# pdishuck/GAVISUNK

Measured on NVIDIA B200. Metric: ont_read_gbp_per_s_sunk_matched_validated, higher is better.
Workload: dtype u64

## Files before the change

gavisunk_b200/csrc/probe.cu:

```cuda
#include "table.cuh"
#include <stdlib.h>
#include <vector>

#ifndef PW_WARPS
#define PW_WARPS 8
#endif
#ifndef PW_BLOCKS
#define PW_BLOCKS 4
#endif
#define PW_TILE 512
static_assert(PW_TILE == GVS_TILE_BASES, "ctx.cu sizes the copy segments in probe tiles");
#define PW_RING 64
#define PW_MAXB 32

#define FLAG_KEYERROR 1u
#define FLAG_OVERFLOW 2u

__device__ __forceinline__ u32 p_codes4(u32 x) {
  u32 f = ((x >> 1) ^ (x >> 2)) & 0x03030303u;
  u32 l = x | 0x20202020u;
  u32 letter = __vcmpeq4(l, 0x63636363u) | __vcmpeq4(l, 0x67676767u) | __vcmpeq4(l, 0x74747474u) |
               __vcmpeq4(l, 0x75757575u);
  u32 low = __vcmpeq4(x & 0xFCFCFCFCu, 0u);
  return (f & letter) | (x & low & 0x03030303u);
}
__device__ __forceinline__ u32 p_codes4_fast(u32 x, u32& bad) {
  u32 f = ((x >> 1) ^ (x >> 2)) & 0x03030303u;
  u32 t = f | (f >> 4);
  u32 sel = __byte_perm(t, 0u, 0x4420);
  u32 letters = __byte_perm(0x54474341u, 0u, sel);
  bad |= letters ^ (x & 0xDFDFDFDFu);
  return f;
}
__device__ __forceinline__ u32 p_be8_top(u32 c) { return c * 0x40100401u; }
__device__ __forceinline__ u32 p_gather_top(u32 px, u32 py, u32 pz, u32 pw) {
  u32 t1 = __byte_perm(py, px, 0x0073);
  u32 t2 = __byte_perm(pw, pz, 0x0073);
  return __byte_perm(t2, t1, 0x5410);
}
__device__ __forceinline__ u32 p_pack16_be(uint4 v) {
  return p_gather_top(p_be8_top(p_codes4(v.x)), p_be8_top(p_codes4(v.y)), p_be8_top(p_codes4(v.z)), p_be8_top(p_codes4(v.w)));
}
__device__ __forceinline__ u32 p_pack16_be_fast(uint4 v, u32& bad) {
  return p_gather_top(p_be8_top(p_codes4_fast(v.x, bad)), p_be8_top(p_codes4_fast(v.y, bad)),
                      p_be8_top(p_codes4_fast(v.z, bad)), p_be8_top(p_codes4_fast(v.w, bad)));
}
__device__ __forceinline__ u32 p_rc16(u32 w) {
  u32 x = __brev(~w);
  return ((x >> 1) & 0x55555555u) | ((x & 0x55555555u) << 1);
}
template <int LEN>
__device__ __forceinline__ u64 p_extract(u32 a, u32 b, u32 c, int off) {
  int s = 2 * off;
  u32 hi = __funnelshift_l(b, a, s);
  u32 lo = __funnelshift_l(c, b, s);
  u64 v = ((u64)hi << 32) | lo;
  return v >> (64 - 2 * LEN);
}

struct __align__(16) WarpSmem {
  u32 fw[PW_RING];
  u32 rc[PW_RING];
  uint4 raw[32];
  u64 bar;
  u32 bound[20];
  u32 shrt[20];
  u32 bpos[PW_MAXB];
  u32 bidx[PW_MAXB];
  u32 cand[PW_TILE / 32];
  u16 inv[32];
  u32 q_row[PW_TILE];
  u16 q_p[PW_TILE];
  u32 s_blk[32][3];
  u16 s_p[32];
};

template <int K>
__device__ __forceinline__ u64 p_fwd_at(const WarpSmem& sm, u32 rb, u32 p) {
  u32 wi = rb + (p >> 4);
  return p_extract<K>(sm.fw[wi & 63], sm.fw[(wi + 1) & 63], sm.fw[(wi + 2) & 63], p & 15);
}
template <int K>
__device__ __forceinline__ u64 p_rc_at(const WarpSmem& sm, u32 rb, u32 p) {
  u32 e = p + K, c = (e + 15) >> 4;
  u32 wi = rb + c - 1;
  return p_extract<K>(sm.rc[wi & 63], sm.rc[(wi - 1) & 63], sm.rc[(wi - 2) & 63], 16 * c - e);
}
template <int K>
__device__ __forceinline__ u64 p_canon_at(const WarpSmem& sm, u32 rb, u32 p, bool force_last_a) {
  u64 f = p_fwd_at<K>(sm, rb, p), r = p_rc_at<K>(sm, rb, p);
  if (force_last_a) {
    f &= ~3ull;
    r |= 3ull << (2 * (K - 1));
  }
  return f < r ? f : r;
}

struct Probe2Params {
  const u8* __restrict__ seq;
  u64 total;
  const u64* __restrict__ read_off;
  u64 n_reads;
  u64 tile_begin, tile_stop;
  u64 span_base;
  u32 span_tiles, n_spans;
  u32* span_ctr;
  u32 blk_stream;
  const u32* __restrict__ filt;
  u32 filt_mask;
  const u32* __restrict__ filt1;
  u32 filt1_words;
  TabView tab;
  u32* hit_read;
  u32* hit_w;
  u32* hit_row;
  u32* hit_gidx;
  u8* hit_nf;
  u64 hit_cap;
  u32* flags;
  u32* warp_cnt;
  u64 cap_w;
};

__device__ __forceinline__ u64 p_policy_stream() {
  u64 p;
  asm volatile("createpolicy.fractional.L2::evict_first.b64 %0, 1.0;" : "=l"(p));
  return p;
}
__device__ __forceinline__ u64 p_policy_keep() {
  u64 p;
  asm volatile("createpolicy.fractional.L2::evict_last.b64 %0, 1.0;" : "=l"(p));
  return p;
}
__device__ __forceinline__ uint4 p_ldg_v4(const uint4* ptr, u64 pol) {
  uint4 v;
  asm volatile("ld.global.nc.L2::cache_hint.L2::64B.v4.u32 {%0,%1,%2,%3}, [%4], %5;"
               : "=r"(v.x), "=r"(v.y), "=r"(v.z), "=r"(v.w)
               : "l"(ptr), "l"(pol));
  return v;
}
__device__ __forceinline__ u32 p_ldg_u32(const u32* ptr, u64 pol) {
  u32 v;
  asm volatile("ld.global.nc.L2::cache_hint.L2::64B.u32 %0, [%1], %2;" : "=r"(v) : "l"(ptr), "l"(pol));
  return v;
}

__device__ __forceinline__ u32 p_smem_addr(const void* p) { return (u32)__cvta_generic_to_shared(p); }
__device__ __forceinline__ void p_bar_init(u64* bar) {
  asm volatile("mbarrier.init.shared::cta.b64 [%0], 1;\n" ::"r"(p_smem_addr(bar)) : "memory");
  asm volatile("fence.mbarrier_init.release.cluster;\n" ::: "memory");
}
__device__ __forceinline__ void p_bar_wait(u64* bar, u32 phase) {
  asm volatile(
      "{\n"
      ".reg .pred p;\n"
      "PW_WAIT:\n"
      "mbarrier.try_wait.parity.shared::cta.b64 p, [%0], %1;\n"
      "@p bra PW_DONE;\n"
      "bra PW_WAIT;\n"
      "PW_DONE:\n"
      "}\n" ::"r"(p_smem_addr(bar)),
      "r"(phase)
      : "memory");
}
template <bool PACKED>
__device__ __forceinline__ u32 p_tile_bytes(u64 tile, u64 total) {
  const u64 unit = PACKED ? PW_TILE / 4 : PW_TILE;
  const u64 have = PACKED ? 4 * ((total + 15) >> 4) : total;
  const u64 b0 = tile * unit;
  if (b0 >= have) return 0;
  const u64 r = have - b0;
  return r >= unit ? (u32)unit : (u32)((r + 15) & ~15ull);
}
template <bool PACKED, bool FULL = false>
__device__ __forceinline__ void p_stage_issue(WarpSmem& sm, const u8* __restrict__ seq, u64 tile, u64 total, int lane, u64 pol) {
  const u32 bytes = FULL ? (PACKED ? PW_TILE / 4 : PW_TILE) : p_tile_bytes<PACKED>(tile, total);
  if (lane == 0 && bytes) {
    const u32 bar = p_smem_addr(&sm.bar), dst = p_smem_addr(&sm.raw[0]);
    const u8* src = seq + tile * (PACKED ? PW_TILE / 4 : PW_TILE);
    asm volatile("fence.proxy.async.shared::cta;\n" ::: "memory");
    asm volatile("mbarrier.arrive.expect_tx.shared::cta.b64 _, [%0], %1;\n" ::"r"(bar), "r"(bytes) : "memory");
    asm volatile("cp.async.bulk.shared::cluster.global.mbarrier::complete_tx::bytes.L2::cache_hint [%0], [%1], %2, [%3], %4;\n" ::"r"(dst),
                 "l"(src), "r"(bytes), "r"(bar), "l"(pol)
                 : "memory");
  }
}
template <bool PACKED, bool FULL = false>
__device__ __forceinline__ void p_stage_finish(WarpSmem& sm, u32 rb, u64 tile, u64 total, int lane, u32& phase) {
  if (FULL) {
    p_bar_wait(&sm.bar, phase);
    phase ^= 1u;
    u32 w;
    if (PACKED) {
      w = ((const u32*)sm.raw)[lane];
    } else {
      const uint4 v = sm.raw[lane];
      u32 bad = 0;
      w = p_pack16_be_fast(v, bad);
      if (__any_sync(0xFFFFFFFFu, bad != 0)) w = p_pack16_be(v);
    }
    sm.fw[(rb + lane) & 63] = w;
    sm.rc[(rb + lane) & 63] = p_rc16(w);
    return;
  }
  const u32 bytes = p_tile_bytes<PACKED>(tile, total);
  if (bytes) {
    p_bar_wait(&sm.bar, phase);
    phase ^= 1u;
  }
  u32 w = 0;
  if (PACKED) {
    if (4u * lane < bytes) w = ((const u32*)sm.raw)[lane];
  } else {
    uint4 v = make_uint4(0u, 0u, 0u, 0u);
    const u64 g = tile * PW_TILE + 16ull * lane;
    const bool tail = g + 16 > total;
    if (16u * lane < bytes) {
      v = sm.raw[lane];
      if (tail) {
        const u32 nv = g < total ? (u32)(total - g) : 0u;
        u32 x[4] = {v.x, v.y, v.z, v.w};
#pragma unroll
        for (int i = 0; i < 4; i++) {
          const u32 left = nv > 4u * i ? nv - 4u * i : 0u;
          x[i] &= left >= 4u ? 0xFFFFFFFFu : ((1u << (8 * left)) - 1u);
        }
        v = make_uint4(x[0], x[1], x[2], x[3]);
      }
    }
    u32 bad = 0;
    w = p_pack16_be_fast(v, bad);
    if (__any_sync(0xFFFFFFFFu, (bad != 0) | tail)) w = p_pack16_be(v);
  }
  sm.fw[(rb + lane) & 63] = w;
  sm.rc[(rb + lane) & 63] = p_rc16(w);
}

template <int K, bool PACKED, bool SMALL>
__global__ void __launch_bounds__(PW_WARPS * 32, PW_BLOCKS) k_probe2(const Probe2Params P) {
  __shared__ WarpSmem sm_all[PW_WARPS];
  const int lane = threadIdx.x & 31;
  WarpSmem& sm = sm_all[threadIdx.x >> 5];
  constexpr int CMAX = (K + 15 + 15) / 16;
  constexpr u32 ALL = 0xFFFFFFFFu;
  constexpr int J = GVS_FJ(K);
  constexpr int L = K - J + 1;
  constexpr int NG = 16 / J;
  const u64 pol_keep = p_policy_keep();
  const u64 pol_stream = p_policy_stream();
  const u64 pol_blk = P.blk_stream ? pol_stream : pol_keep;
  if (lane == 0) p_bar_init(&sm.bar);
  __syncwarp();
  u32 phase = 0;

  for (;;) {
    u32 span = 0;
    if (lane == 0) span = atomicAdd(P.span_ctr, 1u);
    span = __shfl_sync(ALL, span, 0);
    if (span >= P.n_spans) break;
    const u64 tile0 = P.tile_begin + (u64)span * P.span_tiles;
    u64 tile_end = tile0 + P.span_tiles;
    if (tile_end > P.tile_stop) tile_end = P.tile_stop;
    const u64 region = P.span_base + span;

    u64 cur;
    {
      u64 ts0 = tile0 * PW_TILE;
      u64 lo = 1, hi = P.n_reads;
      while (lo < hi) {
        u64 mid = (lo + hi) >> 1;
        if (__ldg(P.read_off + mid) > ts0) hi = mid; else lo = mid + 1;
      }
      cur = lo;
    }
    u64 next_off = __ldg(P.read_off + cur);
    u64 prev_off = __ldg(P.read_off + cur - 1);

    __syncwarp();
    p_stage_issue<PACKED>(sm, P.seq, tile0, P.total, lane, pol_stream);
    p_stage_finish<PACKED>(sm, 0, tile0, P.total, lane, phase);
    __syncwarp();
    p_stage_issue<PACKED>(sm, P.seq, tile0 + 1, P.total, lane, pol_stream);
    p_stage_finish<PACKED>(sm, 32, tile0 + 1, P.total, lane, phase);
    __syncwarp();

    const bool span_full = (tile_end + 2) * PW_TILE <= P.total;
    u32 wcount = 0;
    for (u64 tile = tile0; tile < tile_end; tile++) {
      const u64 ts = tile * PW_TILE;
      const u32 rb = (u32)((tile - tile0) & 1) * 32;
      if (span_full) p_stage_issue<PACKED, true>(sm, P.seq, tile + 2, P.total, lane, pol_stream);
      else p_stage_issue<PACKED>(sm, P.seq, tile + 2, P.total, lane, pol_stream);

      const u64 limit = ts + PW_TILE + (K > 1 ? K - 1 : 1);
      const u64 cur0 = cur;
      u32 nb = 0;
      const bool has_bound = next_off < limit;
      const bool start_short = K >= 2 && prev_off == ts && next_off - prev_off == (u64)(K - 1);
      if (has_bound) {
        if (lane < 20) { sm.bound[lane] = 0; sm.shrt[lane] = 0; }
        __syncwarp();
        u64 j = cur + lane;
        for (;;) {
          u64 o = (j <= P.n_reads) ? __ldg(P.read_off + j) : ~0ull;
          bool inr = o < limit;
          bool intile = inr && (o - ts) < PW_TILE;
          u32 bal_tile = __ballot_sync(ALL, intile);
          if (inr) {
            u32 rel = (u32)(o - ts);
            atomicOr(&sm.bound[rel >> 5], 1u << (rel & 31));
            if (intile) {
              u32 slot = nb + __popc(bal_tile & ((1u << lane) - 1));
              if (slot < PW_MAXB) { sm.bpos[slot] = rel; sm.bidx[slot] = (u32)j; }
              if (K >= 2 && j < P.n_reads && __ldg(P.read_off + j + 1) - o == (u64)(K - 1))
                atomicOr(&sm.shrt[rel >> 5], 1u << (rel & 31));
            }
          }
          nb += __popc(bal_tile);
          u32 bal_adv = __ballot_sync(ALL, o <= ts + PW_TILE);
          cur += __popc(bal_adv);
          u32 bal_in = __ballot_sync(ALL, inr);
          if (bal_in != ALL) break;
          j += 32;
        }
        next_off = (cur <= P.n_reads) ? __ldg(P.read_off + cur) : ~0ull;
        prev_off = __ldg(P.read_off + cur - 1);
        __syncwarp();
      }

      u32 cm = 0;
      u32 S16 = 0;
      u32 pass = 0;
      u32 hbv[NG];
      {
        const u32 wb = rb + lane;
        const u32 f0 = sm.fw[wb & 63], f1 = sm.fw[(wb + 1) & 63], f2 = sm.fw[(wb + 2) & 63];
        const u32 r0 = sm.rc[(wb + CMAX - 1) & 63], r1 = sm.rc[(wb + CMAX - 2) & 63], r2 = sm.rc[(wb + CMAX - 3) & 63],
                  r3 = sm.rc[(wb + CMAX - 4) & 63];
        u32 inval = 0;
        if (has_bound) {
          int idx = lane >> 1, sh = (lane & 1) * 16;
          u64 B = ((u64)sm.bound[idx] | ((u64)sm.bound[idx + 1] << 32)) >> sh;
          if (sh) B |= (u64)sm.bound[idx + 2] << 48;
          u64 x = 0;
          if (K >= 2) {
            x = B >> 1;
            int c = 1;
#pragma unroll
            for (int it = 0; it < 6; it++) {
              if (c < K - 1) {
                int step = (K - 1 - c) < c ? (K - 1 - c) : c;
                x |= x >> step;
                c += step;
              }
            }
          }
          inval = (u32)x & 0xFFFFu;
          S16 = (sm.shrt[idx] >> sh) & 0xFFFFu;
        }
        if (start_short && lane == 0) S16 |= 1u;
        {
          u64 p0 = ts + 16ull * lane;
          if (p0 + 16 > P.total) {
            u32 nv = p0 < P.total ? (u32)(P.total - p0) : 0u;
            inval |= 0xFFFFu & ~((1u << nv) - 1);
          }
        }
        sm.inv[lane] = (u16)inval;
        if (lane < PW_TILE / 32) sm.cand[lane] = 0;
        u32 w1[NG];
#pragma unroll
        for (int g = 0; g < NG; g++) {
          const int o = J * g + (J - 1);
          u64 sf = p_extract<L>(f0, f1, f2, o);
          const int e = o + L;
          const int c = (e + 15) / 16;
          const int j0 = CMAX - c;
          const int off = 16 * c - e;
          u64 sr = (j0 == 0) ? p_extract<L>(r0, r1, r2, off) : p_extract<L>(r1, r2, r3, off);
          hbv[g] = gvs_bhash(sf < sr ? sf : sr);
          const u32 gm = (1u << J) - 1;
          const bool any_valid = ((inval >> (J * g)) & gm) != gm;
          w1[g] = any_valid ? p_ldg_u32(P.filt1 + gvs_p1_word(hbv[g], P.filt1_words), pol_keep) : 0u;
        }
#pragma unroll
        for (int g = 0; g < NG; g++)
          pass |= (__funnelshift_r(w1[g], 0u, hbv[g]) & __funnelshift_r(w1[g], 0u, hbv[g] >> 5) & 1u) << g;
      }
      auto read_of = [&](u32 prel) -> u32 {
        if (!has_bound) return (u32)(cur0 - 1);
        if (nb <= PW_MAXB) {
          u32 rd = (u32)(cur0 - 1), bestpos = 0;
          bool any = false;
          for (u32 q = 0; q < nb; q++) {
            u32 bp = sm.bpos[q], bj = sm.bidx[q];
            if (bp <= prel && (!any || bp > bestpos || (bp == bestpos && bj > rd))) {
              any = true;
              bestpos = bp;
              rd = bj;
            }
          }
          return rd;
        }
        u64 p = ts + prel;
        u64 l = 1, h2 = P.n_reads;
        while (l < h2) {
          u64 mid = (l + h2) >> 1;
          if (__ldg(P.read_off + mid) > p) h2 = mid; else l = mid + 1;
        }
        return (u32)(l - 1);
      };
      auto emit_round = [&](u32 row, u32 gi, u32 pp) {
        u32 rd = 0;
        const bool hit = row != GVS_NOHIT;
        const u32 bal = __ballot_sync(ALL, hit);
        if (bal == 0) return;
        if (hit) rd = read_of(pp);
        const u32 below = bal & ((1u << lane) - 1);
        const int prev = below ? 31 - __clz(below) : lane;
        const u32 gi_prev = __shfl_sync(ALL, gi, prev), rd_prev = __shfl_sync(ALL, rd, prev);
        const bool head = hit && (below == 0 || gi != gi_prev || rd != rd_prev);
        const u32 hb = __ballot_sync(ALL, head);
        const u32 nrec = __popc(hb);
        const bool fits = (u64)wcount + nrec <= P.cap_w;
        if (!fits && lane == 0) atomicOr(P.flags, FLAG_OVERFLOW);
        if (head && fits) {
          const u32 above = lane == 31 ? 0u : (hb >> (lane + 1)) << (lane + 1);
          const u32 upto = above ? ((1u << (__ffs(above) - 1)) - 1) : 0xFFFFFFFFu;
          const u32 after = lane == 31 ? 0u : ~((2u << lane) - 1);
          const u64 o = region * P.cap_w + wcount + __popc(hb & ((1u << lane) - 1));
          P.hit_read[o] = rd;
          P.hit_w[o] = (u32)(ts + pp);
          P.hit_row[o] = row;
          P.hit_gidx[o] = gi;
          P.hit_nf[o] = (u8)__popc(bal & upto & after);
        }
        wcount += nrec;
      };
      const bool any_s16 = SMALL && __any_sync(ALL, S16 != 0);
      bool fused = false;
      if (__any_sync(ALL, pass != 0)) {
        const u32 np_lane = __popc(pass);
        u32 incl = np_lane;
#pragma unroll
        for (int d = 1; d < 32; d <<= 1) {
          u32 o = __shfl_up_sync(ALL, incl, d);
          if (lane >= d) incl += o;
        }
        const u32 n_grp = __shfl_sync(ALL, incl, 31);
        u32 qo = incl - np_lane;
#pragma unroll
        for (int g = 0; g < NG; g++) {
          if ((pass >> g) & 1u) {
            sm.q_p[qo] = (u16)(lane * NG + g);
            sm.q_row[qo] = hbv[g];
            qo++;
          }
        }
        __syncwarp();
        const u32 n_ent = n_grp * J;
        constexpr int RB = 2;
        if (SMALL && n_ent <= 32 && !any_s16) {
          u32 row = GVS_NOHIT, gi = 0, p = 0;
          if ((u32)lane < n_ent) {
            const u32 q = lane / J, w = lane % J;
            p = (u32)sm.q_p[q] * J + w;
            const uint4 b4 = p_ldg_v4((const uint4*)P.filt + (sm.q_row[q] & P.filt_mask), pol_blk);
            const bool valid = !((sm.inv[p >> 4] >> (p & 15)) & 1u);
            const u64 canon = p_canon_at<K>(sm, rb, p, false);
            const u32 h = gvs_fhash(canon);
            const u32 t = __funnelshift_r(b4.x, 0u, h) & __funnelshift_r(b4.y, 0u, h >> 5) & __funnelshift_r(b4.z, 0u, h >> 10) &
                          __funnelshift_r(b4.w, 0u, h >> 15);
            if (valid && (t & 1u)) {
              row = tab_lookup(P.tab, canon, gvs_mix(canon), &gi);
              if (row == GVS_ROW_MISSING) {
                atomicOr(P.flags, FLAG_KEYERROR);
                row = GVS_NOHIT;
              } else if (row >= GVS_NOHIT) {
                row = GVS_NOHIT;
              }
            }
          }
          emit_round(row, gi, p);
          fused = true;
        } else if (SMALL) {
        for (u32 base = 0; base < n_ent; base += 32 * RB) {
          uint4 b4[RB];
          u32 pw[RB];
#pragma unroll
          for (int r = 0; r < RB; r++) {
            const u32 e = base + 32 * r + lane;
            pw[r] = 0xFFFFFFFFu;
            b4[r] = make_uint4(0, 0, 0, 0);
            if (e < n_ent) {
              const u32 q = e / J, w = e % J;
              pw[r] = (u32)sm.q_p[q] * J + w;
              b4[r] = p_ldg_v4((const uint4*)P.filt + (sm.q_row[q] & P.filt_mask), pol_blk);
            }
          }
#pragma unroll
          for (int r = 0; r < RB; r++) {
            if (base + 32 * r >= n_ent) break;
            const u32 p = pw[r];
            if (p != 0xFFFFFFFFu) {
              const bool valid = !((sm.inv[p >> 4] >> (p & 15)) & 1u);
              const u32 h = gvs_fhash(p_canon_at<K>(sm, rb, p, false));
              const u32 t = __funnelshift_r(b4[r].x, 0u, h) & __funnelshift_r(b4[r].y, 0u, h >> 5) &
                            __funnelshift_r(b4[r].z, 0u, h >> 10) & __funnelshift_r(b4[r].w, 0u, h >> 15);
              if (valid && (t & 1u)) atomicOr(&sm.cand[p >> 5], 1u << (p & 31));
            }
          }
        }
        } else {
        for (u32 gbase = 0; gbase < n_grp; gbase += 32 * RB) {
          uint4 b4[RB];
          u32 hq[RB];
#pragma unroll
          for (int r = 0; r < RB; r++) {
            const u32 q = gbase + 32 * r + lane;
            hq[r] = 0;
            b4[r] = make_uint4(0, 0, 0, 0);
            if (q < n_grp) {
              hq[r] = sm.q_row[q];
              b4[r] = p_ldg_v4((const uint4*)P.filt + (hq[r] & P.filt_mask), pol_blk);
            }
          }
#pragma unroll
          for (int r = 0; r < RB; r++) {
            if (gbase + 32 * r >= n_grp) break;
            const u32 q = gbase + 32 * r + lane;
            const bool ok = q < n_grp && ((b4[r].w >> gvs_fp_bit(hq[r])) & 1u);
            const u32 bal = __ballot_sync(ALL, ok);
            if (bal == 0) continue;
            if (ok) {
              const u32 slot = __popc(bal & ((1u << lane) - 1));
              sm.s_p[slot] = sm.q_p[q];
              sm.s_blk[slot][0] = b4[r].x;
              sm.s_blk[slot][1] = b4[r].y;
              sm.s_blk[slot][2] = b4[r].z;
            }
            __syncwarp();
            const u32 n_win = __popc(bal) * J;
            for (u32 base = 0; base < n_win; base += 32) {
              const u32 e = base + lane;
              if (e < n_win) {
                const u32 sq = e / J, w = e % J;
                const u32 p = (u32)sm.s_p[sq] * J + w;
                const bool valid = !((sm.inv[p >> 4] >> (p & 15)) & 1u);
                const u32 h = gvs_fhash(p_canon_at<K>(sm, rb, p, false));
                const u32 t = __funnelshift_r(sm.s_blk[sq][0], 0u, h) & __funnelshift_r(sm.s_blk[sq][1], 0u, h >> 5) &
                              __funnelshift_r(sm.s_blk[sq][2], 0u, h >> 10);
                if (valid && (t & 1u)) atomicOr(&sm.cand[p >> 5], 1u << (p & 31));
              }
            }
            __syncwarp();
          }
        }
        }
        __syncwarp();
        if (!fused) cm = (sm.cand[lane >> 1] >> ((lane & 1) * 16)) & 0xFFFFu;
      }
      if (S16) {
        for (u32 s16 = S16; s16; s16 &= s16 - 1) {
          int i = __ffs(s16) - 1;
          u32 p = 16u * lane + i;
          u64 canon = p_canon_at<K>(sm, rb, p, true);
          u64 sub = (p_fwd_at<K>(sm, rb, p) & ~3ull) >> (2 * (K - L));
          u64 subr = gvs_revcomp(sub, L);
          uint4 b4 = __ldg((const uint4*)P.filt + (gvs_bhash(sub < subr ? sub : subr) & P.filt_mask));
          u32 h = gvs_fhash(canon);
          u32 t = __funnelshift_r(b4.x, 0u, h) & __funnelshift_r(b4.y, 0u, h >> 5) & __funnelshift_r(b4.z, 0u, h >> 10);
          if (SMALL) t &= __funnelshift_r(b4.w, 0u, h >> 15);
          if (t & 1u) cm |= 1u << i; else cm &= ~(1u << i);
        }
      }
      cm |= (S16 << 16);
      if (__any_sync(ALL, (cm & 0xFFFFu) != 0)) {
        u32 ncand_lane = __popc(cm & 0xFFFFu);
        u32 incl = ncand_lane;
#pragma unroll
        for (int d = 1; d < 32; d <<= 1) {
          u32 o = __shfl_up_sync(ALL, incl, d);
          if (lane >= d) incl += o;
        }
        const u32 ncand = __shfl_sync(ALL, incl, 31);
        u32 qo = incl - ncand_lane;
        for (u32 s = cm & 0xFFFFu; s; s &= s - 1) {
          int i = __ffs(s) - 1;
          sm.q_p[qo++] = (u16)((16u * lane + i) | (((cm >> (16 + i)) & 1) << 15));
        }
        __syncwarp();
        for (u32 base = 0; base < ncand; base += 32) {
          u32 row = GVS_NOHIT, gi = 0;
          u32 pp = 0;
          if (base + lane < ncand) {
            u32 e = sm.q_p[base + lane];
            pp = e & 0x7FFFu;
            u64 canon = p_canon_at<K>(sm, rb, pp, (e >> 15) != 0);
            row = tab_lookup(P.tab, canon, gvs_mix(canon), &gi);
            if (row == GVS_ROW_MISSING) {
              atomicOr(P.flags, FLAG_KEYERROR);
              row = GVS_NOHIT;
            } else if (row >= GVS_NOHIT) {
              row = GVS_NOHIT;
            }
          }
          emit_round(row, gi, pp);
        }
      }
      __syncwarp();
      if (span_full) p_stage_finish<PACKED, true>(sm, rb, tile + 2, P.total, lane, phase);
      else p_stage_finish<PACKED>(sm, rb, tile + 2, P.total, lane, phase);
      __syncwarp();
    }
    if (lane == 0) P.warp_cnt[region] = wcount;
  }
}

typedef void (*probe_fn)(const Probe2Params);
static probe_fn probe_table(int k, bool packed, bool small) {
  switch (k) {
#ifdef GVS_PROBE_ONLY_K
#define PK(n) case n: if (n != GVS_PROBE_ONLY_K) return nullptr; return packed ? (small ? k_probe2<GVS_PROBE_ONLY_K, true, true> : k_probe2<GVS_PROBE_ONLY_K, true, false>) \
                                    : (small ? k_probe2<GVS_PROBE_ONLY_K, false, true> : k_probe2<GVS_PROBE_ONLY_K, false, false>);
#else
#define PK(n) case n: return packed ? (small ? k_probe2<n, true, true> : k_probe2<n, true, false>) \
                                    : (small ? k_probe2<n, false, true> : k_probe2<n, false, false>);
#endif
    PK(1) PK(2) PK(3) PK(4) PK(5) PK(6) PK(7) PK(8) PK(9) PK(10) PK(11) PK(12) PK(13) PK(14) PK(15) PK(16)
    PK(17) PK(18) PK(19) PK(20) PK(21) PK(22) PK(23) PK(24) PK(25) PK(26) PK(27) PK(28) PK(29) PK(30) PK(31)
#undef PK
  }
  return nullptr;
}

int gvs_probe_launch(gvs_ctx* ctx, u64* n_warps_out, u64* cap_w_out) {
  u64 total = ctx->total_bases;
  u64 n_tiles = cdiv(total, PW_TILE);
  probe_fn fn = probe_table(ctx->k, ctx->seq_packed, !ctx->filt_fp);
  if (!fn) return gvs_fail(ctx, GVS_E_ARG, "no probe kernel for k=%d", ctx->k);
  u64* counters = ctx->counters.as<u64>();
  Probe2Params P;
  P.seq = ctx->seq;
  P.total = total;
  P.read_off = ctx->read_off;
  P.n_reads = ctx->n_reads;
  struct Seg { u64 t0, t1, span_base, ev; u32 span_tiles, n_spans, blocks; };
  std::vector<Seg> plan;
  const bool piped = !ctx->seg_tile_end.empty() && ctx->seq == ctx->own_seq.as<u8>();
  const u64 n_launch = piped ? ctx->seg_tile_end.size() : 1;
  const u64 resident_warps = (u64)ctx->n_sm * PW_BLOCKS * PW_WARPS;
  u64 spans = 0;
  for (u64 s = 0, t0 = 0; s < n_launch; s++) {
    u64 t1 = piped ? ctx->seg_tile_end[s] : n_tiles;
    if (t1 > t0) {
      u64 st = cdiv(t1 - t0, resident_warps * 32);
      if (st < 8) st = 8;
      if (st > 1024) st = 1024;
      u64 ns = cdiv(t1 - t0, st);
      u64 blocks = cdiv(ns, PW_WARPS);
      if (blocks > (u64)ctx->n_sm * PW_BLOCKS) blocks = (u64)ctx->n_sm * PW_BLOCKS;
      plan.push_back({t0, t1, spans, s, (u32)st, (u32)ns, (u32)blocks});
      spans += ns;
    }
    t0 = t1;
  }
  if (spans >= 0xFFFFFFF0ull) return gvs_fail(ctx, GVS_E_OVERFLOW, "too many probe spans");
  *n_warps_out = spans;
  CKR(gvs_reserve(ctx, ctx->tile_cnt, spans * 4));
  CKR(gvs_reserve(ctx, ctx->tile_dst, spans * 8));
  CKR(gvs_reserve(ctx, ctx->tile_off, (plan.size() + 1) * 4));
  CK(cudaMemsetAsync(ctx->tile_cnt.p, 0, spans * 4, ctx->stream));
  CK(cudaMemsetAsync(ctx->tile_off.p, 0, (plan.size() + 1) * 4, ctx->stream));
  P.cap_w = ctx->hit_cap / spans;
  *cap_w_out = P.cap_w;
  P.filt = ctx->filt.as<u32>();
  P.filt_mask = (u32)(ctx->filt_words - 1);
  P.filt1 = ctx->filt1.as<u32>();
  P.filt1_words = (u32)ctx->filt1_words;
  P.blk_stream = ctx->filt_words * 16 > (32ull << 20) ? 1u : 0u;
  P.tab.kv = ctx->tab_kv.as<u64>();
  P.tab.slots = ctx->tab_slots;
  P.hit_read = ctx->hit_read.as<u32>();
  P.hit_w = ctx->hit_w.as<u32>();
  P.hit_row = ctx->hit_row.as<u32>();
  P.hit_gidx = ctx->hit_gidx.as<u32>();
  P.hit_nf = ctx->hit_nf.as<u8>();
  P.hit_cap = ctx->hit_cap;
  P.flags = (u32*)(counters + 1);
  P.warp_cnt = ctx->tile_cnt.as<u32>();
  if (ctx->l2_persist_max < 0) {
    cudaDeviceGetAttribute(&ctx->l2_persist_max, cudaDevAttrMaxPersistingL2CacheSize, ctx->device);
    cudaDeviceGetAttribute(&ctx->l2_window_max, cudaDevAttrMaxAccessPolicyWindowSize, ctx->device);
    if (ctx->l2_persist_max < 0) ctx->l2_persist_max = 0;
  }
  const int persist_max = ctx->l2_persist_max, window_max = ctx->l2_window_max;
  {
    static bool said = false;
    if (!said && getenv("GVS_EXP_VERBOSE")) {
      said = true;
      fprintf(stderr, "[gvs] L2 persisting max %d B, access window max %d B, presence filter %llu B, block filter %llu B, table %llu slots\n",
              persist_max, window_max, (unsigned long long)ctx->filt1_words * 4, (unsigned long long)ctx->filt_words * 16,
              (unsigned long long)ctx->tab_slots);
    }
  }
  const void* hot = ctx->filt1.p;
  size_t hot_bytes = ctx->filt1_words * 4;
  cudaLaunchConfig_t cfg = {};
  cfg.blockDim = dim3(PW_WARPS * 32);
  cfg.dynamicSmemBytes = 0;
  cfg.stream = ctx->stream;
  cudaLaunchAttribute attr[1];
  int n_attr = 0;
  static const int exp_no_persist = getenv("GVS_EXP_NO_PERSIST") ? atoi(getenv("GVS_EXP_NO_PERSIST")) : 0;
  if (persist_max > 0 && window_max > 0 && exp_no_persist != 1) {
    size_t carve = hot_bytes < (size_t)persist_max ? hot_bytes : (size_t)persist_max;
    if (exp_no_persist == 2) carve = (size_t)persist_max;
    if (ctx->l2_carve_set != carve) {
      cudaDeviceSetLimit(cudaLimitPersistingL2CacheSize, carve);
      ctx->l2_carve_set = carve;
    }
    size_t win = hot_bytes < (size_t)window_max ? hot_bytes : (size_t)window_max;
    attr[0].id = cudaLaunchAttributeAccessPolicyWindow;
    attr[0].val.accessPolicyWindow.base_ptr = const_cast<void*>(hot);
    attr[0].val.accessPolicyWindow.num_bytes = win;
    attr[0].val.accessPolicyWindow.hitRatio = win <= carve ? 1.0f : (float)carve / (float)win;
    attr[0].val.accessPolicyWindow.hitProp = cudaAccessPropertyPersisting;
    attr[0].val.accessPolicyWindow.missProp = cudaAccessPropertyStreaming;
    n_attr = 1;
  }
  cfg.attrs = attr;
  cfg.numAttrs = n_attr;
  for (size_t s = 0; s < plan.size(); s++) {
    probe_fn fn_s = fn;
    P.seq = ctx->seq;
    if (piped) {
      CKR(gvs_pipe_wait(ctx, plan[s].ev));
      if (!ctx->seg_packed.empty() && ctx->seg_packed[plan[s].ev]) {
        fn_s = probe_table(ctx->k, true, !ctx->filt_fp);
        P.seq = ctx->own_words.as<u8>();
      }
      CK(cudaStreamWaitEvent(ctx->stream, ctx->seg_ev[plan[s].ev], 0));
    }
    cfg.gridDim = dim3(plan[s].blocks);
    P.tile_begin = plan[s].t0;
    P.tile_stop = plan[s].t1;
    P.span_tiles = plan[s].span_tiles;
    P.n_spans = plan[s].n_spans;
    P.span_base = plan[s].span_base;
    P.span_ctr = ctx->tile_off.as<u32>() + s;
    cudaError_t e = cudaLaunchKernelEx(&cfg, fn_s, P);
    ctx->launches++;
    if (e == cudaSuccess) e = cudaGetLastError();
    if (e != cudaSuccess) return gvs_fail(ctx, GVS_E_CUDA, "k_probe2 launch: %s", cudaGetErrorString(e));
  }
  if (piped) CKR(gvs_pipe_join(ctx));
  return 0;
}
```

Measured before the change: 394.5.

## Batch probe candidates across tiles into full-warp lookup rounds and shrink q_row

Candidate canonical k-mers from the general lookup path are now staged in a per-warp shared queue (key, position, read) and drained only when 32 are collected or at span end. Previously each tile issued a partially filled warp round of hash lookups. Batching keeps every lane busy during the random table access. The q_row buffer is sized by the group count (PW_TILE/J) to cut shared memory, with a static assert on the carve-out. The risk is extra shared-memory stores and read_of calls for candidates that never hit, plus drain checks before the fused path.

```diff
diff --git a/gavisunk_b200/csrc/probe.cu b/gavisunk_b200/csrc/probe.cu
--- a/gavisunk_b200/csrc/probe.cu
+++ b/gavisunk_b200/csrc/probe.cu
@@ -58,36 +58,40 @@
   return v >> (64 - 2 * LEN);
 }
 
+template <int NGRP>
 struct __align__(16) WarpSmem {
   u32 fw[PW_RING];
   u32 rc[PW_RING];
   uint4 raw[32];
   u64 bar;
+  u64 c_key[32];
+  u32 c_pos[32];
+  u32 c_read[32];
   u32 bound[20];
   u32 shrt[20];
   u32 bpos[PW_MAXB];
   u32 bidx[PW_MAXB];
   u32 cand[PW_TILE / 32];
   u16 inv[32];
-  u32 q_row[PW_TILE];
+  u32 q_row[NGRP];
   u16 q_p[PW_TILE];
   u32 s_blk[32][3];
   u16 s_p[32];
 };
 
-template <int K>
-__device__ __forceinline__ u64 p_fwd_at(const WarpSmem& sm, u32 rb, u32 p) {
+template <int K, class SM>
+__device__ __forceinline__ u64 p_fwd_at(const SM& sm, u32 rb, u32 p) {
   u32 wi = rb + (p >> 4);
   return p_extract<K>(sm.fw[wi & 63], sm.fw[(wi + 1) & 63], sm.fw[(wi + 2) & 63], p & 15);
 }
-template <int K>
-__device__ __forceinline__ u64 p_rc_at(const WarpSmem& sm, u32 rb, u32 p) {
+template <int K, class SM>
+__device__ __forceinline__ u64 p_rc_at(const SM& sm, u32 rb, u32 p) {
   u32 e = p + K, c = (e + 15) >> 4;
   u32 wi = rb + c - 1;
   return p_extract<K>(sm.rc[wi & 63], sm.rc[(wi - 1) & 63], sm.rc[(wi - 2) & 63], 16 * c - e);
 }
-template <int K>
-__device__ __forceinline__ u64 p_canon_at(const WarpSmem& sm, u32 rb, u32 p, bool force_last_a) {
+template <int K, class SM>
+__device__ __forceinline__ u64 p_canon_at(const SM& sm, u32 rb, u32 p, bool force_last_a) {
   u64 f = p_fwd_at<K>(sm, rb, p), r = p_rc_at<K>(sm, rb, p);
   if (force_last_a) {
     f &= ~3ull;
@@ -172,8 +176,8 @@
   const u64 r = have - b0;
   return r >= unit ? (u32)unit : (u32)((r + 15) & ~15ull);
 }
-template <bool PACKED, bool FULL = false>
-__device__ __forceinline__ void p_stage_issue(WarpSmem& sm, const u8* __restrict__ seq, u64 tile, u64 total, int lane, u64 pol) {
+template <bool PACKED, bool FULL = false, class SM>
+__device__ __forceinline__ void p_stage_issue(SM& sm, const u8* __restrict__ seq, u64 tile, u64 total, int lane, u64 pol) {
   const u32 bytes = FULL ? (PACKED ? PW_TILE / 4 : PW_TILE) : p_tile_bytes<PACKED>(tile, total);
   if (lane == 0 && bytes) {
     const u32 bar = p_smem_addr(&sm.bar), dst = p_smem_addr(&sm.raw[0]);
@@ -185,8 +189,8 @@
                  : "memory");
   }
 }
-template <bool PACKED, bool FULL = false>
-__device__ __forceinline__ void p_stage_finish(WarpSmem& sm, u32 rb, u64 tile, u64 total, int lane, u32& phase) {
+template <bool PACKED, bool FULL = false, class SM>
+__device__ __forceinline__ void p_stage_finish(SM& sm, u32 rb, u64 tile, u64 total, int lane, u32& phase) {
   if (FULL) {
     p_bar_wait(&sm.bar, phase);
     phase ^= 1u;
@@ -238,12 +242,14 @@
 
 template <int K, bool PACKED, bool SMALL>
 __global__ void __launch_bounds__(PW_WARPS * 32, PW_BLOCKS) k_probe2(const Probe2Params P) {
-  __shared__ WarpSmem sm_all[PW_WARPS];
+  constexpr int J = GVS_FJ(K);
+  static_assert(J < 4 || PW_BLOCKS * (PW_WARPS * sizeof(WarpSmem<PW_TILE / J>) + 1024) <= 132 * 1024,
+                "probe shared memory beyond the 132 KB carve-out: L1 shrinks and the probe slows down");
+  __shared__ WarpSmem<PW_TILE / J> sm_all[PW_WARPS];
   const int lane = threadIdx.x & 31;
-  WarpSmem& sm = sm_all[threadIdx.x >> 5];
+  auto& sm = sm_all[threadIdx.x >> 5];
   constexpr int CMAX = (K + 15 + 15) / 16;
   constexpr u32 ALL = 0xFFFFFFFFu;
-  constexpr int J = GVS_FJ(K);
   constexpr int L = K - J + 1;
   constexpr int NG = 16 / J;
   const u64 pol_keep = p_policy_keep();
@@ -286,6 +292,50 @@
 
     const bool span_full = (tile_end + 2) * PW_TILE <= P.total;
     u32 wcount = 0;
+    u32 qn = 0;
+    auto emit_round = [&](u32 row, u32 gi, u32 w, u32 rd) {
+      const bool hit = row != GVS_NOHIT;
+      const u32 bal = __ballot_sync(ALL, hit);
+      if (bal == 0) return;
+      const u32 below = bal & ((1u << lane) - 1);
+      const int prev = below ? 31 - __clz(below) : lane;
+      const u32 gi_prev = __shfl_sync(ALL, gi, prev), rd_prev = __shfl_sync(ALL, rd, prev);
+      const bool head = hit && (below == 0 || gi != gi_prev || rd != rd_prev);
+      const u32 hb = __ballot_sync(ALL, head);
+      const u32 nrec = __popc(hb);
+      const bool fits = (u64)wcount + nrec <= P.cap_w;
+      if (!fits && lane == 0) atomicOr(P.flags, FLAG_OVERFLOW);
+      if (head && fits) {
+        const u32 above = lane == 31 ? 0u : (hb >> (lane + 1)) << (lane + 1);
+        const u32 upto = above ? ((1u << (__ffs(above) - 1)) - 1) : 0xFFFFFFFFu;
+        const u32 after = lane == 31 ? 0u : ~((2u << lane) - 1);
+        const u64 o = region * P.cap_w + wcount + __popc(hb & ((1u << lane) - 1));
+        P.hit_read[o] = rd;
+        P.hit_w[o] = w;
+        P.hit_row[o] = row;
+        P.hit_gidx[o] = gi;
+        P.hit_nf[o] = (u8)__popc(bal & upto & after);
+      }
+      wcount += nrec;
+    };
+    auto drain = [&]() {
+      u32 row = GVS_NOHIT, gi = 0, w = 0, rd = 0;
+      if ((u32)lane < qn) {
+        const u64 canon = sm.c_key[lane];
+        w = sm.c_pos[lane];
+        rd = sm.c_read[lane];
+        row = tab_lookup(P.tab, canon, gvs_mix(canon), &gi);
+        if (row == GVS_ROW_MISSING) {
+          atomicOr(P.flags, FLAG_KEYERROR);
+          row = GVS_NOHIT;
+        } else if (row >= GVS_NOHIT) {
+          row = GVS_NOHIT;
+        }
+      }
+      __syncwarp();
+      emit_round(row, gi, w, rd);
+      qn = 0;
+    };
     for (u64 tile = tile0; tile < tile_end; tile++) {
       const u64 ts = tile * PW_TILE;
       const u32 rb = (u32)((tile - tile0) & 1) * 32;
@@ -410,33 +460,6 @@
         }
         return (u32)(l - 1);
       };
-      auto emit_round = [&](u32 row, u32 gi, u32 pp) {
-        u32 rd = 0;
-        const bool hit = row != GVS_NOHIT;
-        const u32 bal = __ballot_sync(ALL, hit);
-        if (bal == 0) return;
-        if (hit) rd = read_of(pp);
-        const u32 below = bal & ((1u << lane) - 1);
-        const int prev = below ? 31 - __clz(below) : lane;
-        const u32 gi_prev = __shfl_sync(ALL, gi, prev), rd_prev = __shfl_sync(ALL, rd, prev);
-        const bool head = hit && (below == 0 || gi != gi_prev || rd != rd_prev);
-        const u32 hb = __ballot_sync(ALL, head);
-        const u32 nrec = __popc(hb);
-        const bool fits = (u64)wcount + nrec <= P.cap_w;
-        if (!fits && lane == 0) atomicOr(P.flags, FLAG_OVERFLOW);
-        if (head && fits) {
-          const u32 above = lane == 31 ? 0u : (hb >> (lane + 1)) << (lane + 1);
-          const u32 upto = above ? ((1u << (__ffs(above) - 1)) - 1) : 0xFFFFFFFFu;
-          const u32 after = lane == 31 ? 0u : ~((2u << lane) - 1);
-          const u64 o = region * P.cap_w + wcount + __popc(hb & ((1u << lane) - 1));
-          P.hit_read[o] = rd;
-          P.hit_w[o] = (u32)(ts + pp);
-          P.hit_row[o] = row;
-          P.hit_gidx[o] = gi;
-          P.hit_nf[o] = (u8)__popc(bal & upto & after);
-        }
-        wcount += nrec;
-      };
       const bool any_s16 = SMALL && __any_sync(ALL, S16 != 0);
       bool fused = false;
       if (__any_sync(ALL, pass != 0)) {
@@ -461,6 +484,7 @@
         const u32 n_ent = n_grp * J;
         constexpr int RB = 2;
         if (SMALL && n_ent <= 32 && !any_s16) {
+          if (qn) drain();
           u32 row = GVS_NOHIT, gi = 0, p = 0;
           if ((u32)lane < n_ent) {
             const u32 q = lane / J, w = lane % J;
@@ -481,7 +505,7 @@
               }
             }
           }
-          emit_round(row, gi, p);
+          emit_round(row, gi, (u32)(ts + p), row != GVS_NOHIT ? read_of(p) : 0u);
           fused = true;
         } else if (SMALL) {
         for (u32 base = 0; base < n_ent; base += 32 * RB) {
@@ -590,22 +614,18 @@
           sm.q_p[qo++] = (u16)((16u * lane + i) | (((cm >> (16 + i)) & 1) << 15));
         }
         __syncwarp();
-        for (u32 base = 0; base < ncand; base += 32) {
-          u32 row = GVS_NOHIT, gi = 0;
-          u32 pp = 0;
-          if (base + lane < ncand) {
-            u32 e = sm.q_p[base + lane];
-            pp = e & 0x7FFFu;
-            u64 canon = p_canon_at<K>(sm, rb, pp, (e >> 15) != 0);
-            row = tab_lookup(P.tab, canon, gvs_mix(canon), &gi);
-            if (row == GVS_ROW_MISSING) {
-              atomicOr(P.flags, FLAG_KEYERROR);
-              row = GVS_NOHIT;
-            } else if (row >= GVS_NOHIT) {
-              row = GVS_NOHIT;
-            }
-          }
-          emit_round(row, gi, pp);
+        for (u32 base = 0; base < ncand;) {
+          const u32 n = ncand - base < 32 - qn ? ncand - base : 32 - qn;
+          if ((u32)lane < n) {
+            const u32 e = sm.q_p[base + lane], pp = e & 0x7FFFu;
+            sm.c_key[qn + lane] = p_canon_at<K>(sm, rb, pp, (e >> 15) != 0);
+            sm.c_pos[qn + lane] = (u32)(ts + pp);
+            sm.c_read[qn + lane] = read_of(pp);
+          }
+          __syncwarp();
+          qn += n;
+          base += n;
+          if (qn == 32) drain();
         }
       }
       __syncwarp();
@@ -613,6 +633,7 @@
       else p_stage_finish<PACKED>(sm, rb, tile + 2, P.total, lane, phase);
       __syncwarp();
     }
+    if (qn) drain();
     if (lane == 0) P.warp_cnt[region] = wcount;
   }
 }
diff --git a/profiles/probe_stage.py b/profiles/probe_stage.py
--- /dev/null
+++ b/profiles/probe_stage.py
@@ -0,0 +1,64 @@
+import argparse
+import json
+import os
+import subprocess
+import sys
+
+import numpy as np
+
+ROOT = os.path.dirname(os.path.dirname(os.path.abspath(__file__)))
+sys.path.insert(0, ROOT)
+
+
+def gpu_info():
+    try:
+        out = subprocess.run(["nvidia-smi", "--query-gpu=name,power.limit,clocks.max.sm", "--format=csv,noheader", "-i", "0"],
+                             capture_output=True, text=True, timeout=20).stdout.strip()
+    except Exception as ex:
+        out = f"nvidia-smi unavailable: {ex}"
+    return out
+
+
+def main():
+    ap = argparse.ArgumentParser()
+    ap.add_argument("--lib", default=None, help="library to measure (default: the package's own build)")
+    ap.add_argument("--batches", type=int, default=2)
+    ap.add_argument("--passes", type=int, default=12)
+    ap.add_argument("--tag", default="")
+    a = ap.parse_args()
+    if a.lib:
+        os.environ["GVS_LIB_PATH"] = os.path.abspath(a.lib)
+    import torch
+    from gavisunk_b200 import workload as W
+    from gavisunk_b200 import _lib
+    from gavisunk_b200.engine import Engine
+    if not torch.cuda.is_available():
+        raise SystemExit("probe_stage.py measures on a GPU; none found")
+    eng = Engine(20)
+    contigs = W.human_contigs(3100.0)
+    wl = W.make_assembly(eng, contigs, snp_rate=1e-3, dup_frac=0.01, seed=1001, name="h3100")
+    W.build_db(eng, wl)
+    batch_args = dict(coverage=3.75, n50=100000.0, sigma=0.8, len_min=1000, len_max=1000000, nchunks=10)
+    batches = [W.new_batch(eng, wl, seed=2001 + 16 * b, **batch_args) for b in range(a.batches)]
+    binds = [(lambda e, b=b: W.bind_batch(e, b)) for b in batches]
+    eng.set_profiling(True)
+    ms, rows = [], []
+
+    def on_batch(e, b, base):
+        ms.append(e.stage_ms("probe"))
+        rows.append(int(e.n_rows))
+    eng.run_batches(binds, wl.contig_hap)
+    for _ in range(a.passes):
+        eng.run_batches(binds, wl.contig_hap, on_batch=on_batch)
+    ms = np.array(ms)
+    print(json.dumps(dict(
+        metric="probe_ms_per_launch", tag=a.tag, lib=_lib.LIB_PATH,
+        workload=f"h3100 (bench.py default: 3.1 Gbp x2, k 20), first {a.batches} batches of 3.75x, reads resident as ASCII, 1 GPU",
+        gpu=gpu_info(), launches=int(len(ms)), bases_per_batch=[int(b.read_off[-1].item()) for b in batches],
+        rows_per_batch=rows[:a.batches], rows_same_every_pass=all(r == rows[j % a.batches] for j, r in enumerate(rows)),
+        probe_ms_median=float(np.median(ms)), probe_ms_min=float(ms.min()), probe_ms_max=float(ms.max()))))
+    eng.close()
+
+
+if __name__ == "__main__":
+    main()
```

Measured after the change: 422.4, median of 6. +7.1%, better.
